# santi-pdp/segan_pytorch

Hardware: AMD Instinct MI355X
Metric: 16384-sample waveform chunks/sec (GAN step) (higher is better)
Workload: dtype f32

## Files before the change

include/segan_hip.h:

```cpp
#ifndef SEGAN_HIP_H
#define SEGAN_HIP_H

#include <stddef.h>
#include <stdint.h>

#ifdef __cplusplus
extern "C" {
#endif

#define SEGAN_ABI_VERSION 13

#define SEGAN_PAD_REFLECT 0
#define SEGAN_PAD_ZERO 1

#define SEGAN_ACT_NONE 0
#define SEGAN_ACT_TANH 1

typedef struct segan_src {
  const float* p0;
  const float* p1;
  int32_t C0;
  int32_t C1;
  const float* scale;
  const float* shift;
  const float* slope;
} segan_src;

int segan_abi_version(void);
const char* segan_last_error(void);

int segan_set_reserved_slots(int n);

size_t segan_packed_f_bytes(int M, int N, int S);
// ... 82 lines not shown
int segan_gemm(const float* A, int64_t sam, int64_t sak, const float* B, int64_t sbk, int64_t sbn,
               float* C, int64_t ldc, int M, int N, int K, int beta0, int flags, void* scratch,
               size_t scratch_bytes, void* stream);

int segan_bias_prelu_rows(const float* x, const float* bias, const float* slope, float* y,
                          int rows, int cols, void* stream);
int segan_bias_prelu_rows_bwd(const float* x, const float* bias, const float* slope,
                              const float* dy, float* dx, float* dslope, float* dbias, int rows,
                              int cols, void* stream);

int segan_mse_const(const float* x, float target, float* loss, float* grad, const float* gout,
                    float gscale, int n, void* stream);
int segan_bce_logits_const(const float* x, float target, float* loss, float* grad,
                           const float* gout, float gscale, int n, void* stream);
int segan_l1_mean(const float* x, const float* y, float* loss, float* ws, int64_t n,
                  void* stream);
int segan_l1_bwd(const float* x, const float* y, const float* gout, float gscale, float* grad,
                 int64_t n, void* stream);

size_t segan_packed_g_bytes(int M, int N, int S);
int segan_pack_weights_g(const float* w, float* wg, int M, int N, int K, int S, void* stream);
int segan_conv1d_dgrad_short(const float* da, const float* wg, float* dx, int B, int N, int M,
                             int L, int K, int S, int padL, int roll, void* stream);

int segan_pool_time_fwd(const float* x, float* y, int* idx, int rows, int L, int mode,
                        void* stream);
int segan_pool_time_bwd(const float* dy, const int* idx, float* dx, int rows, int L, int mode,
                        void* stream);

int segan_mse_mean(const float* x, const float* y, float* loss, float* ws, int64_t n,
                   void* stream);
int segan_mse_bwd(const float* x, const float* y, const float* gout, float gscale, float* grad,
                  int64_t n, void* stream);

size_t segan_snorm_ws_floats(int A, int Bd, int K, int dim);
int segan_snorm_fwd(const float* w, float* u, float* v, float* w_sn, float* sigma, float* ws, int A,
                    int Bd, int K, int dim, int power_iteration, float eps, void* stream);
int segan_snorm_bwd(const float* dw_sn, const float* w, const float* u, const float* v,
                    const float* sigma, float* dw, float* ws, int A, int Bd, int K, int dim,
                    void* stream);

int segan_stft_pitch(int n_fft);
int segan_stft_basis(float* basis, int n_fft, int win, void* stream);
int segan_stft_frames(const float* x, float* frames, int B, int T, int n_fft, int hop, int win,
                      void* stream);
int segan_powdb(const float* S, float* db, int64_t rows, int nbins, int pitch, float eps,
// ... 36 lines not shown
```

segan_pytorch_amd/_lib.py:

```python
import ctypes
import os
from ctypes import POINTER, Structure, c_char_p, c_double, c_float, c_int, c_int32, c_int64, c_size_t, c_void_p

_HERE = os.path.dirname(os.path.abspath(__file__))
LIB_PATH = os.environ.get('SEGAN_HIP_LIB') or os.path.join(_HERE, 'libsegan_hip.so')

PAD_REFLECT = 0
PAD_ZERO = 1
ACT_NONE = 0
ACT_TANH = 1
ABI_VERSION = 13


class SeganSrc(Structure):
    _fields_ = [('p0', c_void_p), ('p1', c_void_p), ('C0', c_int32), ('C1', c_int32),
                ('scale', c_void_p), ('shift', c_void_p), ('slope', c_void_p)]


_P = c_void_p
_SRC = POINTER(SeganSrc)

SIGNATURES = {
    'segan_abi_version': (c_int, []),
    'segan_set_reserved_slots': (c_int, [c_int]),
    'segan_last_error': (c_char_p, []),
    'segan_packed_f_bytes': (c_size_t, [c_int, c_int, c_int]),
    'segan_packed_t_bytes': (c_size_t, [c_int, c_int, c_int]),
    'segan_pack_weights': (c_int, [_P, _P, _P, c_int, c_int, c_int, c_int, c_int, _P]),
    'segan_packed_bf_bytes': (c_size_t, [c_int, c_int, c_int, c_int, c_int]),
    'segan_pack_weights_bf': (c_int, [_P, _P, c_int, c_int, c_int, c_int, c_int, c_int, c_int, _P]),
    'segan_corr_scratch_bytes': (c_size_t, []),
    'segan_bf16_scratch_bytes': (c_size_t, [c_int] * 9),
    'segan_debug_last_corr': (None, [POINTER(c_int)]),
    'segan_debug_last_wgrad': (None, [POINTER(c_int)]),
# ... 14 lines not shown
    'segan_bn_partial': (c_int, [_P, _P, c_int, c_int, c_int, _P]),
    'segan_bn_final': (c_int, [_P, c_int, _P, _P, c_float, c_float, _P, _P, _P, _P, _P, _P, c_int, _P]),
    'segan_act_bwd_bn_reduce': (c_int, [_P] * 12 + [c_int, c_int, c_int, _P]),
    'segan_act_bwd_bn_apply': (c_int, [_P] * 11 + [c_int, c_int, c_int, c_double, _P]),
    'segan_affine_prelu': (c_int, [_P, _P, _P, _P, _P, c_int, c_int, c_int, _P]),
    'segan_affine_tanh': (c_int, [_P, _P, _P, _P, c_int, c_int, c_int, _P]),
    'segan_scale_mask': (c_int, [_P, _P, _P, _P, c_int, c_int, c_int, _P]),
    'segan_sum_skip': (c_int, [_P, _P, _P, _P, _P, c_int, c_int, c_int, _P]),
    'segan_bce_logits_const': (c_int, [_P, c_float, _P, _P, _P, c_float, c_int, _P]),
    'segan_act_bwd': (c_int, [_P] * 16 + [c_int, c_int, c_int, _P]),
    'segan_tanh_bwd': (c_int, [_P, _P, _P, c_float, _P, _P, _P, c_int, c_int, c_int, _P]),
    'segan_gemm_scratch_bytes': (c_size_t, [c_int, c_int, c_int]),
    'segan_gemm': (c_int, [_P, c_int64, c_int64, _P, c_int64, c_int64, _P, c_int64, c_int, c_int,
                           c_int, c_int, c_int, _P, c_size_t, _P]),
    'segan_bias_prelu_rows': (c_int, [_P, _P, _P, _P, c_int, c_int, _P]),
    'segan_bias_prelu_rows_bwd': (c_int, [_P, _P, _P, _P, _P, _P, _P, c_int, c_int, _P]),
    'segan_mse_const': (c_int, [_P, c_float, _P, _P, _P, c_float, c_int, _P]),
    'segan_l1_bwd': (c_int, [_P, _P, _P, c_float, _P, c_int64, _P]),
    'segan_l1_mean': (c_int, [_P, _P, _P, _P, c_int64, _P]),
    'segan_packed_g_bytes': (c_size_t, [c_int, c_int, c_int]),
    'segan_pack_weights_g': (c_int, [_P, _P, c_int, c_int, c_int, c_int, _P]),
    'segan_conv1d_dgrad_short': (c_int, [_P, _P, _P, c_int, c_int, c_int, c_int, c_int, c_int, c_int,
                                        c_int, _P]),
    'segan_pool_time_fwd': (c_int, [_P, _P, _P, c_int, c_int, c_int, _P]),
    'segan_pool_time_bwd': (c_int, [_P, _P, _P, c_int, c_int, c_int, _P]),
    'segan_mse_mean': (c_int, [_P, _P, _P, _P, c_int64, _P]),
    'segan_mse_bwd': (c_int, [_P, _P, _P, c_float, _P, c_int64, _P]),
    'segan_snorm_ws_floats': (c_size_t, [c_int, c_int, c_int, c_int]),
    'segan_snorm_fwd': (c_int, [_P, _P, _P, _P, _P, _P, c_int, c_int, c_int, c_int, c_int, c_float, _P]),
    'segan_snorm_bwd': (c_int, [_P, _P, _P, _P, _P, _P, _P, c_int, c_int, c_int, c_int, _P]),
    'segan_pcm16_prep': (c_int, [_P, _P, _P, _P, c_int, c_int, c_double, _P]),
    'segan_stft_basis': (c_int, [_P, c_int, c_int, _P]),
    'segan_stft_frames': (c_int, [_P, _P, c_int, c_int, c_int, c_int, c_int, _P]),
    'segan_stft_pitch': (c_int, [c_int]),
    'segan_powdb': (c_int, [_P, _P, c_int64, c_int, c_int, c_float, _P]),
    'segan_powdb_bwd': (c_int, [_P, _P, _P, c_int64, c_int, c_int, c_float, _P]),
    'segan_stft_overlap_add': (c_int, [_P, _P, c_int, c_int, c_int, c_int, c_int, _P]),
    'segan_deemphasis': (c_int, [_P, _P, c_int, c_int, c_double, _P]),
    'segan_ssnr_frames': (c_int, [c_int, c_int]),
    'segan_ssnr': (c_int, [_P, _P, _P, _P, c_int, c_int, c_int, c_double, _P]),
    'segan_rmsprop_step': (c_int, [_P, _P, _P, c_float, c_float, c_float, c_int64, _P]),
    'segan_adam_step': (c_int, [_P, _P, _P, _P, c_float, c_float, c_float, c_float, c_int, c_int64,
                                _P]),
    'segan_fill': (c_int, [_P, c_float, c_int64, _P]),
    'segan_scale': (c_int, [_P, c_float, c_int64, _P]),
    'segan_comm_id_bytes': (c_int, []),
# ... 46 lines not shown
```

segan_pytorch_amd/csrc/segan_common.h:

```cpp
#pragma once
#include <hip/hip_runtime.h>
#include <stdint.h>
#include <stdio.h>
#include <stdarg.h>
#include "../../include/segan_hip.h"

#define SEGAN_OK 0
#define SEGAN_EINVAL (-1)
#define SEGAN_ELAUNCH (-2)
#define SEGAN_EUNSUPPORTED (-3)

void segan_set_error(const char* fmt, ...);
int segan_check_launch(const char* what);

#define SEGAN_REQUIRE(cond, ...)                 \
  do {                                           \
    if (!(cond)) {                               \
      segan_set_error(__VA_ARGS__);              \
      return SEGAN_EINVAL;                       \
    }                                            \
  } while (0)

typedef float f32x16 __attribute__((ext_vector_type(16)));
typedef float f32x4 __attribute__((ext_vector_type(4)));
// ... 42 lines not shown
  float sc, sh, sl;
};

__device__ __forceinline__ ChanXf segan_chan_xf(const segan_src& s, int c) {
  ChanXf x;
  x.sc = s.scale[c];
  x.sh = s.shift[c];
  x.sl = s.slope[c];
  return x;
}

__device__ __forceinline__ float segan_apply_xf(const ChanXf& x, float v) {
  v = fmaf(v, x.sc, x.sh);
  return v > 0.0f ? v : v * x.sl;
}

int segan_src_defaults(segan_src* s, hipStream_t st, const char* what);

__device__ __forceinline__ const float* segan_src_row(const segan_src& s, int b, int n, int L) {
  if (n < s.C0) return s.p0 + ((size_t)b * s.C0 + n) * (size_t)L;
  return s.p1 + ((size_t)b * s.C1 + (n - s.C0)) * (size_t)L;
}

__device__ __forceinline__ float warp_sum(float v) {
#pragma unroll
  for (int o = 32; o > 0; o >>= 1) v += __shfl_down(v, o, 64);
  return v;
}
```

segan_pytorch_amd/csrc/segan_conv.hip:

```cpp
#include "segan_conv_shared.h"

template <int MB, int NB, int WM, int U>
struct TileGeom {
  static constexpr int S = 32 / U;
  static constexpr int WN = 4 / WM;
  static constexpr int NI = MB / (32 * WM);
  static constexpr int NJ = NB / (32 * WN);
  static constexpr int NPT = MB / S;
};

struct TileWork {
  int tile, c0, c1;
  bool partial;
  int piece;
};

struct TileIter {
  int tileA;
  long unit, unit_end;
  int first_tile;
  __device__ __forceinline__ void init(const CorrArgs& a, int nch) {
    tileA = blockIdx.x;
    unit = (long)blockIdx.x * a.sk_units;
    unit_end = min(unit + (long)a.sk_units, a.sk_total);
// ... 886 lines not shown
    return;
  }
  const int row = blockIdx.x * blockDim.x + threadIdx.x;
  if (row >= rows) return;
  float* d = dx + (size_t)row * L;
  const float* hrow = halo + (size_t)row * hl;
  for (int P = 0; P < padL; ++P) {
    const int idx = segan_hi_index(P, L, padL, SEGAN_PAD_REFLECT, roll);
    if (idx >= 0) d[idx] += hrow[P];
  }
  for (int P2 = 0; P2 < padR; ++P2) {
    const int idx = segan_hi_index(L + padL + P2, L, padL, SEGAN_PAD_REFLECT, roll);
    if (idx >= 0) d[idx] += hrow[padL + P2];
  }
}

#define CS_KC 16
struct ShortArgs {
  const float* da;
  const float* wg;
  float* dx;
  int B, N, M, L, Ls, padL, padRw, roll, ncoltiles;
  int xr8, xbc;
};

template <int S>
__global__ __launch_bounds__(256, 2) void conv_dgrad_short_kernel(const ShortArgs a) {
  constexpr int MB = 128, NB = 128, KC = CS_KC, NI = 2, NJ = 2, YP = 65, U = 32 / S;
  extern __shared__ __attribute__((aligned(16))) float smem[];
  float* Wl0 = smem;
  float* Il0 = smem + 2 * KC * MB;
  const int tid = threadIdx.x;
  const int lane = tid & 63;
  const int wave = __builtin_amdgcn_readfirstlane(tid >> 6);
  const int wm = wave >> 1, wn = wave & 1;
  const int l31 = lane & 31, h = lane >> 5;
  int rowtile, coltile;
  if (a.xbc > 0) {
    const int x = blockIdx.x & 7, k = blockIdx.x >> 3;
    const int per = a.xr8 * a.xbc;
    const int cb = k / per, rem = k - cb * per;
    const int wdt = min(a.xbc, a.ncoltiles - cb * a.xbc);
    const int rr = rem / wdt;
    rowtile = x * a.xr8 + rr;
    coltile = cb * a.xbc + rem - rr * wdt;
  } else {
    const int vb = xcd_remap(blockIdx.x, gridDim.x);
    rowtile = vb / a.ncoltiles;
    coltile = vb - rowtile * a.ncoltiles;
// ... 30 lines not shown

  int aoff[NI], boff[NJ], rsh[NI];
#pragma unroll
  for (int i = 0; i < NI; ++i) {
    aoff[i] = h * MB + 32 * (wm * NI + i) + l31;
    rsh[i] = 0;
  }
#pragma unroll
  for (int j = 0; j < NJ; ++j) boff[j] = h * NB + 64 * wn + 32 * j + l31;

  f32x16 acc[NI][NJ];
#pragma unroll
  for (int i = 0; i < NI; ++i)
#pragma unroll
    for (int j = 0; j < NJ; ++j)
#pragma unroll
      for (int e = 0; e < 16; ++e) acc[i][j][e] = 0.0f;

  const int nch = a.M / KC;
  float b30_unused[NJ] = {};
  load_chunk(0, 0);
  __builtin_amdgcn_s_waitcnt(0x0f70);
  __syncthreads();
  for (int ch = 0; ch < nch; ++ch) {
    const int buf = ch & 1;
    if (ch + 1 < nch) load_chunk(ch + 1, buf ^ 1);
    corr_mma_chunk<MB, 1, KC, NI, NJ, false>(Wl0 + buf * (KC * MB), Il0 + buf * (KC * NB), NB, aoff,
                                             boff, rsh, acc, b30_unused, h, aoff, boff);
    __builtin_amdgcn_s_waitcnt(0x0f70);
    __syncthreads();
  }

  float* Yb = smem + wave * (32 * YP);
  const int bw = b0 + (64 * wn) / Ls;
  auto dxp = [&](int P, int cbase) -> float {
    const int r = P % S, qq = P / S;
    float v = 0.0f;
#pragma unroll
    for (int u = 0; u < U; ++u) {
      const int t = qq - u;
      if (t >= 0 && t < Ls) v += Yb[(r * U + u) * YP + cbase + t];
    }
    return v;
  };
#pragma unroll
  for (int i = 0; i < NI; ++i) {
#pragma unroll
    for (int j = 0; j < NJ; ++j)
#pragma unroll
      for (int e = 0; e < 16; ++e)
        Yb[((e & 3) + 8 * (e >> 2) + 4 * h) * YP + 32 * j + l31] = acc[i][j][e];
    __syncthreads();
    const int n = n0 + 2 * wm + i;
#pragma unroll
    for (int p = 0; p < S; ++p) {
      const int o = p * 64 + lane;
      const int sl = o / L, io = o - sl * L;
      const int b = bw + sl;
      float v = dxp(io + a.padL, sl * Ls);
      if (io >= 1 && io <= a.padL) v += dxp(a.padL - io, sl * Ls);
      const int jr = L - 2 - io;
      if (jr >= 0 && jr < a.padRw) v += dxp(L + a.padL + jr, sl * Ls);
      if (b < a.B && n < a.N) {
        int ii = io - a.roll;
        if (ii < 0) ii += L;
        if (ii >= L) ii -= L;
        a.dx[((size_t)b * a.N + n) * L + ii] = v;
      }
    }
    __syncthreads();
  }
}

__global__ void pack_g_kernel(const float* __restrict__ w, float* __restrict__ wg, int M, int N,
                              int K, int S) {
  const size_t total = (size_t)M * N * 32;
  const int U = 32 / S;
  for (size_t i = blockIdx.x * (size_t)blockDim.x + threadIdx.x; i < total;
       i += (size_t)gridDim.x * blockDim.x) {
    const int c = (int)(i & 31);
    const size_t mn = i >> 5;
    const int k = S * (c % U) + c / U;
    wg[i] = k < K ? w[mn * K + k] : 0.0f;
  }
}

static thread_local int g_last_corr[6];
void segan_note_corr_launch(int kind, unsigned grid, const CorrArgs& a, int ntiles) {
  g_last_corr[0] = kind;
  g_last_corr[1] = (int)grid;
  g_last_corr[2] = ntiles;
  g_last_corr[3] = a.sk_nfull;
  g_last_corr[4] = a.sk_total > 0 ? a.sk_units : 0;
// ... 463 lines not shown
  if (!stride_ok(S) || L % S != 0) return false;
  const int Ls = L / S;
  return (Ls == 4 || Ls == 8 || Ls == 16 || Ls == 32 || Ls == 64) && N % 4 == 0 &&
         M % CS_KC == 0 && K >= 1 && K <= 32 && padL >= 0 && K - 1 - padL >= 0 && padL < L &&
         K - S - padL < L;
}

extern "C" size_t segan_packed_g_bytes(int M, int N, int S) {
  if (!stride_ok(S) || M <= 0 || N <= 0) return 0;
  return (size_t)M * N * 32 * sizeof(float);
}

extern "C" int segan_pack_weights_g(const float* w, float* wg, int M, int N, int K, int S,
                                    void* stream) {
  SEGAN_REQUIRE(w && wg && M > 0 && N > 0, "pack_weights_g: bad arguments");
  SEGAN_REQUIRE(stride_ok(S) && K >= 1 && K <= 32, "pack_weights_g: stride in {1,2,4}, K <= 32");
  const size_t total = (size_t)M * N * 32;
  const int blocks = (int)((total + 255) / 256 > 8192 ? 8192 : (total + 255) / 256);
  hipLaunchKernelGGL(pack_g_kernel, dim3(blocks), dim3(256), 0, (hipStream_t)stream, w, wg, M, N, K,
                     S);
  return segan_check_launch("pack_weights_g");
}

extern "C" int segan_conv1d_dgrad_short(const float* da, const float* wg, float* dx, int B, int N,
                                        int M, int L, int K, int S, int padL, int roll,
                                        void* stream) {
  SEGAN_REQUIRE(da && wg && dx && B > 0, "conv1d_dgrad_short: bad arguments");
  SEGAN_REQUIRE(roll > -L && roll < L, "conv1d_dgrad_short: |roll| must be < L");
  if (!short_ok(N, M, L, K, S, padL)) {
    segan_set_error("conv1d_dgrad_short: geometry not covered (L/S in {4,8,16,32,64}, N %% 4 == 0, "
                    "M %% 16 == 0)");
    return SEGAN_EUNSUPPORTED;
  }
  ShortArgs a;
  a.da = da; a.wg = wg; a.dx = dx;
  a.B = B; a.N = N; a.M = M; a.L = L; a.Ls = L / S; a.padL = padL;
  a.padRw = K - S - padL > 0 ? K - S - padL : 0;
  a.roll = roll;
  a.ncoltiles = ceil_div(B, 128 / a.Ls);
  const size_t lds = 4 * 32 * 65 * sizeof(float);
  const dim3 grid((unsigned)(N / 4 * a.ncoltiles));
  static const bool blocked = [] {
    const char* e = getenv("SEGAN_SHORT_ORDER");
    return !(e && e[0] == '0');
  }();
  a.xr8 = a.xbc = 0;
  if (blocked && (N / 4) % 8 == 0) {
    a.xr8 = N / 4 / 8;
    a.xbc = a.xr8 >= 128 ? 1 : 128 / a.xr8;
  }
  hipStream_t st = (hipStream_t)stream;
  if (S == 4) hipLaunchKernelGGL(conv_dgrad_short_kernel<4>, grid, dim3(256), lds, st, a);
  else if (S == 2) hipLaunchKernelGGL(conv_dgrad_short_kernel<2>, grid, dim3(256), lds, st, a);
  else hipLaunchKernelGGL(conv_dgrad_short_kernel<1>, grid, dim3(256), lds, st, a);
  return segan_check_launch("conv_dgrad_short_kernel");
}
```

segan_pytorch_amd/csrc/segan_pointwise.hip:

```cpp
#include "segan_common.h"

#define PW_THREADS 256

static int pw_nsplit(int B, int C, int L) {
  int ns = ceil_div(2048, C);
  if (ns > B) ns = B;
  long per = (long)B * L / ns;
  while (ns > 1 && per < 2048) {
    ns = (ns + 1) / 2;
    per = (long)B * L / ns;
  }
  return ns < 1 ? 1 : ns;
}

extern "C" int segan_bn_nsplit(int B, int C, int L) {
  if (B <= 0 || C <= 0 || L <= 0) return 0;
  return pw_nsplit(B, C, L);
}

template <int NV>
__device__ __forceinline__ void block_sum(float (&v)[NV], float* sm) {
  const int lane = threadIdx.x & 63, wave = threadIdx.x >> 6;
#pragma unroll
  for (int k = 0; k < NV; ++k) v[k] = warp_sum(v[k]);
// ... 77 lines not shown
    const float r = s1 / n;
    mean = K + r;
    m2 = fmaxf(s2 - s1 * r, 0.0f);
  }
#pragma unroll
  for (int o = 32; o > 0; o >>= 1) {
    const float nb2 = __shfl_down(n, o, 64), mb2 = __shfl_down(mean, o, 64), qb2 = __shfl_down(m2, o, 64);
    chan_combine(n, mean, m2, nb2, mb2, qb2);
  }
  const int lane = threadIdx.x & 63, wave = threadIdx.x >> 6;
  if (lane == 0) {
    sm[3 * wave] = n; sm[3 * wave + 1] = mean; sm[3 * wave + 2] = m2;
  }
  __syncthreads();
  if (threadIdx.x == 0) {
    for (int w = 1; w < PW_THREADS / 64; ++w) chan_combine(n, mean, m2, sm[3 * w], sm[3 * w + 1], sm[3 * w + 2]);
    float* w = ws + ((size_t)blockIdx.y * C + cr.c) * 3;
    w[0] = n;
    w[1] = mean;
    w[2] = m2;
  }
}

__device__ __forceinline__ void bn_affine(float gamma, float beta, float mean, float rstd,
                                          float& scale, float& shift) {
  scale = gamma * rstd;
  shift = fmaf(-mean, scale, beta);
}

__global__ void bn_final_kernel(const float* __restrict__ ws, const float* gamma, const float* beta,
                                float eps, float momentum, float* running_mean, float* running_var,
                                float* mean_o, float* rstd_o, float* scale_o, float* shift_o, int C,
                                int nsplit) {
  const int c = blockIdx.x * blockDim.x + threadIdx.x;
  if (c >= C) return;
  double n = 0.0, mean = 0.0, m2 = 0.0;
  for (int s = 0; s < nsplit; ++s) {
    const float* w = ws + ((size_t)s * C + c) * 3;
    const double nb = w[0], mb = w[1], qb = w[2];
    if (nb <= 0.0) continue;
    const double tot = n + nb;
    const double d = mb - mean;
    mean += d * nb / tot;
    m2 += qb + d * d * n * nb / tot;
    n = tot;
  }
  const double var = n > 0 ? m2 / n : 0.0;
  const float rstd = (float)(1.0 / sqrt(var + (double)eps));
  const float g = gamma ? gamma[c] : 1.0f;
  const float bt = beta ? beta[c] : 0.0f;
  float sc, sh;
// ... 761 lines not shown
```

segan_pytorch_amd/distributed.py:

```python
import os
import time

import torch
import torch.distributed as dist

from . import ops


def is_dist():
    return dist.is_available() and dist.is_initialized() and dist.get_world_size() > 1


def world_size():
    return dist.get_world_size() if (dist.is_available() and dist.is_initialized()) else 1


def _collectives_on():
    if not (dist.is_available() and dist.is_initialized()):
        return False
    return dist.get_world_size() > 1 or os.environ.get('SEGAN_DP_SINGLE') == '1'


def rank():
    return dist.get_rank() if (dist.is_available() and dist.is_initialized()) else 0
# ... 436 lines not shown
    if n % ws != 0:
        raise ValueError('global batch {} is not divisible by world size {}'.format(n, ws))
    per = n // ws
    return t.narrow(dim, rk * per, per)


def sync_bn_enabled():
    return _collectives_on() and os.environ.get("SEGAN_SYNC_BN", "0") == "1"


def bn_stats_sync(x, gamma, beta, eps, momentum, running_mean, running_var):
    ws = ops.bn_partial(x)
    if _native_cur is not None:
        allp = _native_cur.allgather(ws).view(-1, ws.shape[1], 3)
    else:
        parts = [torch.empty_like(ws) for _ in range(world_size())]
        dist.all_gather(parts, ws)
        allp = torch.cat(parts, 0).contiguous()
    return ops.bn_final(allp, gamma, beta, eps, momentum, running_mean, running_var)


def act_bwd_bn_sync(a, dh, slope, bn, dslope=None, dgamma=None, dbeta=None, dbias=None):
    totals, ws = ops.act_bwd_bn_reduce(a, dh, slope, bn, dslope, dgamma, dbeta)
    if _native_cur is not None:
        _native_cur.allreduce(totals, 1.0)
    else:
        dist.all_reduce(totals, op=dist.ReduceOp.SUM)
    count = float(a.shape[0]) * float(a.shape[2]) * world_size()
    return ops.act_bwd_bn_apply(a, dh, slope, bn, totals, count, dbias, ws)
```

segan_pytorch_amd/functional.py:

```python
import os

import torch

from . import ops
from .ops import ACT_NONE, ACT_TANH, PAD_REFLECT, PAD_ZERO, Src


def grad_buf(p):
    if p.grad is None:
        p.grad = torch.zeros_like(p, memory_format=torch.contiguous_format)
    elif not p.grad.is_contiguous():
        p.grad = p.grad.contiguous()
    return p.grad


def _gb(p, needed=True):
    if p is None or not needed or not p.requires_grad:
        return None
    return grad_buf(p)


def _bn_batch_stats(bn, training):
    return training or bn.running_mean is None or bn.running_var is None

# ... 18 lines not shown
    rstd = torch.rsqrt(bn.running_var + bn.eps)
    gamma = bn.weight.detach() if bn.weight is not None else torch.ones_like(rstd)
    beta = bn.bias.detach() if bn.bias is not None else torch.zeros_like(rstd)
    scale = (gamma * rstd).contiguous()
    shift = (beta - bn.running_mean * scale).contiguous()
    return scale, shift, rstd.contiguous()


def _eval_bn_act_bwd(c, bn, scale, shift, rstd, dh, slope, dslope, y_tanh=None, dbias=None):
    if y_tanh is not None:
        g = ops.tanh_bwd(y_tanh, dh, dbias=_gb(bn.bias))
    else:
        v = ops.affine_prelu(c, scale, shift, None)
        g = ops.act_bwd(v, dh, slope=slope, dslope=dslope, dbias=_gb(bn.bias))
    if bn.weight is not None and bn.weight.requires_grad:
        xhat = ops.affine_prelu(c, rstd, (-bn.running_mean * rstd).contiguous(), None)
        grad_buf(bn.weight).add_((g * xhat).sum((0, 2)))
    dc = ops.affine_prelu(g, scale, None, None)
    if dbias is not None:
        ops.act_bwd(dc, dc, dbias=dbias)
    return dc


def _act_bwd_bn(a, dh, slope, bn, dslope, dgamma, dbeta, dbias):
    from . import distributed as sdist
    if sdist.sync_bn_enabled():
        return sdist.act_bwd_bn_sync(a, dh, slope, bn, dslope, dgamma, dbeta, dbias)
    return ops.act_bwd(a, dh, slope=slope, bn=bn, dslope=dslope, dgamma=dgamma, dbeta=dbeta,
                       dbias=dbias)


_WGRAD_OVERLAP = os.environ.get('SEGAN_WGRAD_OVERLAP', '0') == '1'
_side_streams = {}


class _SideStream(object):

    def __init__(self, *tensors):
        flat = []
        for t in tensors:
            if isinstance(t, Src):
                flat.extend((t.t0, t.t1, t.scale, t.shift, t.slope))
            else:
                flat.append(t)
        self.tensors = [t for t in flat if torch.is_tensor(t) and t.is_cuda]
        self.on = _WGRAD_OVERLAP and bool(self.tensors)

    def __enter__(self):
        if not self.on:
            return self
        dev = self.tensors[0].device
        main = torch.cuda.current_stream(dev)
# ... 323 lines not shown
                _ready(blk)
            if is_conv:
                d_in = ops.conv1d_dgrad(da, w, src.L, S, pack=blk._pack)
                if li == 0:
                    dh_last_enc = d_in if gen.no_z else d_in[:, src.C0:].contiguous()
                else:
                    dh = d_in
            elif li == 0:
                if gen.no_z:
                    _d0, dh_last_enc = ops.deconv1d_dgrad(da, w, S, 0, pack=blk._pack)
                else:
                    _d0, dh_last_enc = ops.deconv1d_dgrad(da, w, S, src.C0, need0=False,
                                                          pack=blk._pack)
            else:
                if src.C1 > 0:
                    dh, dsk = ops.deconv1d_dgrad(da, w, S, src.C0, pack=blk._pack)
                    dskip[n_enc - 1 - li] = dsk
                else:
                    _d0, dh = ops.deconv1d_dgrad(da, w, S, 0, pack=blk._pack)
                    if getattr(src, 'sum_of', False):
                        dskip[n_enc - 1 - li] = dh
        dh = dh_last_enc
        dx = None
        for l in range(n_enc - 1, -1, -1):
            blk = enc[l]
            w = W.get(blk.conv)
            K, S = blk.kwidth, blk.stride
            bnsv = bn_enc[l]
            bnm = getattr(blk, 'norm', None)
            sc, sh = xf_enc[l]
            gskip = gen.skips[l]['alpha'] if (gen.skip and l in gen.skips) else None
            dsk = dskip.get(l)
            mask, a_norm = skip_saved.get(l, (None, None))
            if dsk is not None and mask is not None:
                dsk = ops.scale_mask(dsk, None, mask)
            alpha_p = None
            if gskip is not None and gskip.skip_type == 'conv':
                if dsk is not None:
                    dsk = _skip_conv_bwd(gskip, dsk, Src(a_enc[l], scale=sc, shift=sh), W)
                alpha_v = _ones(a_enc[l].shape[1], a_enc[l]) if dsk is not None else None
                ready_extra = gskip.skip_k
            else:
                alpha_p = gskip.skip_k if gskip is not None else None
                alpha_v = alpha_p if dsk is not None else None
                ready_extra = alpha_p
            if bnsv is None:
                da = ops.act_bwd(a_enc[l], dh, dskip=dsk, slope=blk.act.weight, alpha=alpha_v,
                                 dslope=_gb(blk.act.weight),
                                 dalpha=_gb(alpha_p, dsk is not None),
                                 dbias=_gb(blk.conv.bias))
            elif dsk is None:
                da = _act_bwd_bn(a_enc[l], dh, blk.act.weight, bnsv, _gb(blk.act.weight),
                                 _gb(bnm.weight), _gb(bnm.bias), _gb(blk.conv.bias))
            else:
                if a_norm is None:
                    a_norm = ops.affine_prelu(a_enc[l], sc, sh, None)
                g = ops.act_bwd(a_norm, dh, dskip=dsk, slope=blk.act.weight, alpha=alpha_v,
                                dslope=_gb(blk.act.weight), dalpha=_gb(alpha_p, True))
                da = _act_bwd_bn(a_enc[l], g, None, bnsv, None, _gb(bnm.weight), _gb(bnm.bias),
                                 _gb(blk.conv.bias))
            padL = ops.conv_pad(K, S)[0]
            with _SideStream(da, src_enc[l]):
                if W.needs_grad(blk.conv):
                    gw = W.grad_target(blk.conv)
                    ops.wgrad(Src(da), src_enc[l], gw, K, S, padL, PAD_REFLECT)
                    W.finish(blk.conv, gw)
                _ready(blk, ready_extra)
            if l > 0:
                dh = ops.conv1d_dgrad(da, w, src_enc[l].L, S, pack=blk._pack)
            elif ctx.x_needs:
                dx = ops.conv1d_dgrad(da, w, src_enc[l].L, S, pack=blk._pack)
        _join_side(dy)
        ctx.state = None
        return (None, None, dx, None) + (None,) * (len(ctx.needs_input_grad) - 4)


class DiscriminatorFn(torch.autograd.Function):

    @staticmethod
    def forward(ctx, disc, rolls, x, x1, *params):
        x = x.contiguous()
        blocks = list(disc.enc_blocks)
        training = disc.training
        src = Src(x) if x1 is None else Src(x, x1.contiguous())
        cs, srcs, bns, xfs = [], [], [], []
        W = _Weights()
        for l, blk in enumerate(blocks):
            c = ops.conv1d_fwd(src, W.get(blk.conv), blk.conv.bias, blk.stride, roll=rolls[l],
                               pack=blk._pack)
            srcs.append(src)
            cs.append(c)
            if blk.norm is not None:
# ... 78 lines not shown
            dh = ops.linear_dgrad(dy1, W.get(fc[0])).view(cs[-1].shape)
            _ready(fc)
        else:
            h, hp, idx, y3 = head
            Lh = h.shape[2]
            dy3 = ops.bias_prelu_rows_bwd(y3, fc.bias, None, dout, None, _gb(fc.bias))
            lin_wgrad(fc, dy3, hp)
            dhp = ops.linear_dgrad(dy3, W.get(fc))
            if disc.pool_type == 'conv':
                pcm = disc.pool_conv
                dpc = dhp.view(h.shape[0], 1, Lh)
                if pcm.bias is not None and pcm.bias.requires_grad:
                    ops.act_bwd(dpc, dpc, dbias=grad_buf(pcm.bias))
                if W.needs_grad(pcm):
                    gw = W.grad_target(pcm)
                    ops.wgrad(Src(dpc), Src(h), gw, 1, 1, 0, PAD_ZERO)
                    W.finish(pcm, gw)
                dh = ops.conv1d_dgrad(dpc, W.get(pcm), Lh, 1, padL=0, pack=disc._pool_pack)
                _ready(fc, pcm)
            else:
                dh = ops.pool_time_bwd(dhp, idx, Lh, 'max' if disc.pool_type == 'gmax' else 'avg')
                _ready(fc)
        dx = None
        for l in range(len(blocks) - 1, -1, -1):
            blk = blocks[l]
            w = W.get(blk.conv)
            K, S = blk.kwidth, blk.stride
            bn = bns[l]
            if bn == 'eval':
                raise RuntimeError('Discriminator backward in eval() mode with BatchNorm is not '
                                   'supported; call .train() (the reference never does this)')
            if bn is not None:
                dc = _act_bwd_bn(cs[l], dh, blk.act.weight, bn, _gb(blk.act.weight), _gb(bn[2]),
                                 _gb(bn[3]), _gb(blk.conv.bias))
            else:
                dc = ops.act_bwd(cs[l], dh, slope=blk.act.weight, dslope=_gb(blk.act.weight),
                                 dbias=_gb(blk.conv.bias))
            padL = ops.conv_pad(K, S)[0]
            with _SideStream(dc, srcs[l]):
                if W.needs_grad(blk.conv):
                    gw = W.grad_target(blk.conv)
                    ops.wgrad(Src(dc), srcs[l], gw, K, S, padL, PAD_REFLECT, roll=ctx.rolls[l])
                    W.finish(blk.conv, gw)
                _ready(blk)
            if l > 0:
                dh = ops.conv1d_dgrad(dc, w, srcs[l].L, S, roll=ctx.rolls[l], pack=blk._pack)
            elif ctx.x_needs:
                dx = ops.conv1d_dgrad(dc, w, srcs[l].L, S, roll=ctx.rolls[l], pack=blk._pack)
        _join_side(dout)
        ctx.state = None
        dx1 = None
        if dx is not None and ctx.split is not None:
            c0, need0, need1 = ctx.split
            dx1 = dx[:, c0:].contiguous() if need1 else None
            dx = dx[:, :c0].contiguous() if need0 else None
        return (None, None, dx, dx1) + (None,) * (len(ctx.needs_input_grad) - 4)


class ConvBlockFn(torch.autograd.Function):

    @staticmethod
    def forward(ctx, blk, x, *params):
        x = x.contiguous()
        src = Src(x)
        W = _Weights()
        c = ops.conv1d_fwd(src, W.get(blk.conv), blk.conv.bias, blk.stride, pack=blk._pack)
        bn_saved = None
        scale = shift = None
        if blk.norm is not None:
# ... 206 lines not shown
```

segan_pytorch_amd/ops.py:

```python
import ctypes

import torch

from . import _lib
from . import layout
from ._lib import ACT_NONE, ACT_TANH, PAD_REFLECT, PAD_ZERO, SeganSrc, check


import os as _os

PREC_FP32, PREC_BF16, PREC_BF16X3 = 0, 1, 3
_PREC_NAMES = {'fp32': PREC_FP32, 'bf16': PREC_BF16, 'bf16x3': PREC_BF16X3}
_precision = _PREC_NAMES[_os.environ.get('SEGAN_PRECISION', 'fp32')]
_EUNSUPPORTED = -3


_deterministic = _os.environ.get('SEGAN_DETERMINISTIC', '0') == '1'


def set_deterministic(on):
    global _deterministic
    _deterministic = bool(on)


# ... 319 lines not shown
    if short_rows_ok(N, M, L, S):
        return conv1d_dgrad_short(da, w, L, S, roll=roll, padL=padL, pack=pack)
    check(lib.segan_conv1d_dgrad(_ptr(da), _ptr(pack.t(w, S, 0)), None, _ptr(dx), _ptr(halo), B, N,
                                 M, L, K, S, padL, roll, _fp32(), *_scratch(), _stream()),
          'conv1d_dgrad')
    return dx


def conv1d_dgrad_short(da, w, L, S, roll=0, padL=None, pack=None):
    _chk(da, 'da', 3)
    _chk(w, 'weight', 3)
    M, N, K = w.shape
    B = da.shape[0]
    if padL is None:
        padL = conv_pad(K, S)[0]
    dx = torch.empty((B, N, L), device=da.device, dtype=torch.float32)
    pack = pack or WeightPack()
    check(_lib.load().segan_conv1d_dgrad_short(_ptr(da), _ptr(pack.g(w, S)), _ptr(dx), B, N,
                                               M, L, K, S, padL, roll, _stream()),
          'conv1d_dgrad_short')
    return dx


_SHORT_LS = (4, 8, 16, 32, 64)


def short_rows_ok(N, M, L, S):
    return S in (2, 4) and L % S == 0 and (L // S) in _SHORT_LS and N % 4 == 0 and M % 16 == 0


def wgrad(lo, hi, dw, K, S, padL, pad_mode, roll=0):
    _chk(dw, 'dw', 3)
    M, N = lo.C, hi.C
    if tuple(dw.shape) != (M, N, K):
        raise ValueError('wgrad: dw {} != ({}, {}, {})'.format(tuple(dw.shape), M, N, K))
    if lo.B != hi.B or lo.L * S != hi.L:
        raise ValueError('wgrad: lo [{}x{}] / hi [{}x{}] inconsistent for stride {}'.format(
            lo.B, lo.L, hi.B, hi.L, S))
    cl, ch = lo.c_struct(), hi.c_struct()
    lib = _lib.load()
    if _precision != PREC_FP32:
        nbytes = lib.segan_wgrad_scratch_bytes(lo.B, M, N, lo.L, S, _precision, 0)
        scratch = _stream_scratch(nbytes, dw.device)
        rc = lib.segan_wgrad(ctypes.byref(cl), ctypes.byref(ch), _ptr(dw), lo.B, M, N, lo.L, K, S,
                             padL, pad_mode, roll, _precision, 0,
                             ctypes.c_void_p(scratch.data_ptr()) if scratch is not None else None,
# ... 564 lines not shown
```

Measured before the change: 3577.

## Fuse PReLU/BatchNorm backward epilogue into short-row dgrad kernel

Adds an epilogue to the short-row transposed-conv dgrad kernel. It applies the previous layer's PReLU (with optional skip tap) or BatchNorm-PReLU backward right after the output is computed. Per-channel partial sums for dslope, dalpha, dbias, dgamma and dbeta are written to a workspace, and a small final kernel reduces them. The encoder and discriminator backward loops now route eligible layers through this path, so the separate activation-backward pass that re-reads the gradient tensor is skipped. In exchange the kernel gains extra register pressure and an extra launch, and it only applies to fp32 short-row shapes.

```diff
diff --git a/include/segan_hip.h b/include/segan_hip.h
--- a/include/segan_hip.h
+++ b/include/segan_hip.h
@@ -8,7 +8,7 @@
 extern "C" {
 #endif
 
-#define SEGAN_ABI_VERSION 13
+#define SEGAN_ABI_VERSION 14
 
 #define SEGAN_PAD_REFLECT 0
 #define SEGAN_PAD_ZERO 1
@@ -137,6 +137,14 @@
 int segan_pack_weights_g(const float* w, float* wg, int M, int N, int K, int S, void* stream);
 int segan_conv1d_dgrad_short(const float* da, const float* wg, float* dx, int B, int N, int M,
                              int L, int K, int S, int padL, int roll, void* stream);
+size_t segan_short_act_ws_floats(int B, int N, int L, int S);
+int segan_conv1d_dgrad_short_act(const float* da, const float* wg, float* dx, int B, int N, int M,
+                                 int L, int K, int S, int padL, int roll, const float* a,
+                                 const float* dskip, const float* slope, const float* alpha,
+                                 const float* bn_mean, const float* bn_rstd,
+                                 const float* bn_gamma, const float* bn_beta, float* dslope,
+                                 float* dalpha, float* dgamma, float* dbeta, float* dbias,
+                                 float* totals, float* ws, void* stream);
 
 int segan_pool_time_fwd(const float* x, float* y, int* idx, int rows, int L, int mode,
                         void* stream);
diff --git a/segan_pytorch_amd/_lib.py b/segan_pytorch_amd/_lib.py
--- a/segan_pytorch_amd/_lib.py
+++ b/segan_pytorch_amd/_lib.py
@@ -9,7 +9,7 @@
 PAD_ZERO = 1
 ACT_NONE = 0
 ACT_TANH = 1
-ABI_VERSION = 13
+ABI_VERSION = 14
 
 
 class SeganSrc(Structure):
@@ -70,6 +70,8 @@
     'segan_pack_weights_g': (c_int, [_P, _P, c_int, c_int, c_int, c_int, _P]),
     'segan_conv1d_dgrad_short': (c_int, [_P, _P, _P, c_int, c_int, c_int, c_int, c_int, c_int, c_int,
                                         c_int, _P]),
+    'segan_short_act_ws_floats': (c_size_t, [c_int, c_int, c_int, c_int]),
+    'segan_conv1d_dgrad_short_act': (c_int, [_P, _P, _P] + [c_int] * 8 + [_P] * 15 + [_P]),
     'segan_pool_time_fwd': (c_int, [_P, _P, _P, c_int, c_int, c_int, _P]),
     'segan_pool_time_bwd': (c_int, [_P, _P, _P, c_int, c_int, c_int, _P]),
     'segan_mse_mean': (c_int, [_P, _P, _P, _P, c_int64, _P]),
diff --git a/segan_pytorch_amd/csrc/segan_common.h b/segan_pytorch_amd/csrc/segan_common.h
--- a/segan_pytorch_amd/csrc/segan_common.h
+++ b/segan_pytorch_amd/csrc/segan_common.h
@@ -88,6 +88,12 @@
   return s.p1 + ((size_t)b * s.C1 + (n - s.C0)) * (size_t)L;
 }
 
+__device__ __forceinline__ void bn_affine(float gamma, float beta, float mean, float rstd,
+                                          float& scale, float& shift) {
+  scale = gamma * rstd;
+  shift = fmaf(-mean, scale, beta);
+}
+
 __device__ __forceinline__ float warp_sum(float v) {
 #pragma unroll
   for (int o = 32; o > 0; o >>= 1) v += __shfl_down(v, o, 64);
diff --git a/segan_pytorch_amd/csrc/segan_conv.hip b/segan_pytorch_amd/csrc/segan_conv.hip
--- a/segan_pytorch_amd/csrc/segan_conv.hip
+++ b/segan_pytorch_amd/csrc/segan_conv.hip
@@ -932,9 +932,11 @@
   float* dx;
   int B, N, M, L, Ls, padL, padRw, roll, ncoltiles;
   int xr8, xbc;
+  const float *ea, *eskip, *eslope, *ealpha, *emean, *erstd, *egamma, *ebeta;
+  float* epart;
 };
 
-template <int S>
+template <int S, int EPI = 0>
 __global__ __launch_bounds__(256, 2) void conv_dgrad_short_kernel(const ShortArgs a) {
   constexpr int MB = 128, NB = 128, KC = CS_KC, NI = 2, NJ = 2, YP = 65, U = 32 / S;
   extern __shared__ __attribute__((aligned(16))) float smem[];
@@ -1011,6 +1013,40 @@
   load_chunk(0, 0);
   __builtin_amdgcn_s_waitcnt(0x0f70);
   __syncthreads();
+  const int bw = b0 + (64 * wn) / Ls;
+  auto out_off = [&](int i, int p) -> long {
+    const int n = n0 + 2 * wm + i;
+    const int o = p * 64 + lane;
+    const int sl = o / L, io = o - sl * L;
+    const int b = bw + sl;
+    if (b >= a.B || n >= a.N) return -1;
+    int ii = io - a.roll;
+    if (ii < 0) ii += L;
+    if (ii >= L) ii -= L;
+    return ((long)b * a.N + n) * L + ii;
+  };
+  float ev[NI][S], ek[NI][S], csl[NI], cal[NI], cmu[NI], crs[NI], csc[NI], csh[NI];
+  auto epi_load = [&]() {
+#pragma unroll
+    for (int i = 0; i < NI; ++i) {
+      const int n = n0 + 2 * wm + i;
+      csl[i] = a.eslope ? a.eslope[n] : 1.0f;
+      cal[i] = a.ealpha ? a.ealpha[n] : 0.0f;
+      cmu[i] = 0.f; crs[i] = 1.f; csc[i] = 1.f; csh[i] = 0.f;
+      if (EPI == 2) {
+        cmu[i] = a.emean[n];
+        crs[i] = a.erstd[n];
+        bn_affine(a.egamma ? a.egamma[n] : 1.0f, a.ebeta ? a.ebeta[n] : 0.0f, cmu[i], crs[i], csc[i],
+                  csh[i]);
+      }
+#pragma unroll
+      for (int p = 0; p < S; ++p) {
+        const long off = out_off(i, p);
+        ev[i][p] = off >= 0 ? a.ea[off] : 0.0f;
+        ek[i][p] = (EPI == 1 && a.eskip && off >= 0) ? a.eskip[off] : 0.0f;
+      }
+    }
+  };
   for (int ch = 0; ch < nch; ++ch) {
     const int buf = ch & 1;
     if (ch + 1 < nch) load_chunk(ch + 1, buf ^ 1);
@@ -1020,8 +1056,8 @@
     __syncthreads();
   }
 
+  if (EPI != 0) epi_load();
   float* Yb = smem + wave * (32 * YP);
-  const int bw = b0 + (64 * wn) / Ls;
   auto dxp = [&](int P, int cbase) -> float {
     const int r = P % S, qq = P / S;
     float v = 0.0f;
@@ -1040,7 +1076,9 @@
       for (int e = 0; e < 16; ++e)
         Yb[((e & 3) + 8 * (e >> 2) + 4 * h) * YP + 32 * j + l31] = acc[i][j][e];
     __syncthreads();
+    if (EPI != 0 && i == 0) __builtin_amdgcn_s_waitcnt(0x0f70);
     const int n = n0 + 2 * wm + i;
+    float r[3] = {0.f, 0.f, 0.f};
 #pragma unroll
     for (int p = 0; p < S; ++p) {
       const int o = p * 64 + lane;
@@ -1054,10 +1092,72 @@
         int ii = io - a.roll;
         if (ii < 0) ii += L;
         if (ii >= L) ii -= L;
+        const float av = ev[i][p];
+        if (EPI == 1) {
+          float g = v * (av > 0.f ? 1.0f : csl[i]);
+          r[0] += v * (av > 0.f ? 0.0f : av);
+          if (a.eskip) {
+            g = fmaf(cal[i], ek[i][p], g);
+            r[1] = fmaf(ek[i][p], av, r[1]);
+          }
+          r[2] += g;
+          v = g;
+        } else if (EPI == 2) {
+          const float xh = (av - cmu[i]) * crs[i];
+          const float vv = fmaf(av, csc[i], csh[i]);
+          const float g = v * (vv > 0.f ? 1.0f : csl[i]);
+          r[0] += v * (vv > 0.f ? 0.0f : vv);
+          r[1] += g;
+          r[2] = fmaf(g, xh, r[2]);
+        }
         a.dx[((size_t)b * a.N + n) * L + ii] = v;
       }
     }
+    if (EPI != 0) {
+#pragma unroll
+      for (int k = 0; k < 3; ++k) r[k] = warp_sum(r[k]);
+      if (lane == 0) {
+        float* w = a.epart + ((size_t)(coltile * 2 + wn) * 3) * a.N + n;
+        w[0] = r[0];
+        w[a.N] = r[1];
+        w[2 * a.N] = r[2];
+      }
+    }
     __syncthreads();
+  }
+}
+
+template <int EPI>
+__global__ __launch_bounds__(256) void short_act_final_kernel(const float* __restrict__ part,
+                                                              int nslots, int N, float* dslope,
+                                                              float* d1, float* d2, float* totals) {
+  __shared__ float sm[3][16][17];
+  const int cl = threadIdx.x & 15, t = threadIdx.x >> 4;
+  const int c = blockIdx.x * 16 + cl;
+  float s[3] = {0.f, 0.f, 0.f};
+  if (c < N)
+    for (int k = t; k < nslots; k += 16)
+#pragma unroll
+      for (int q = 0; q < 3; ++q) s[q] += part[((size_t)k * 3 + q) * N + c];
+#pragma unroll
+  for (int q = 0; q < 3; ++q) sm[q][t][cl] = s[q];
+  __syncthreads();
+  for (int w = 8; w > 0; w >>= 1) {
+    if (t < w)
+#pragma unroll
+      for (int q = 0; q < 3; ++q) sm[q][t][cl] += sm[q][t + w][cl];
+    __syncthreads();
+  }
+  if (t != 0 || c >= N) return;
+#pragma unroll
+  for (int q = 0; q < 3; ++q) s[q] = sm[q][0][cl];
+  const float o0 = dslope ? dslope[c] : 0.f, o1 = d1 ? d1[c] : 0.f, o2 = d2 ? d2[c] : 0.f;
+  if (dslope) dslope[c] = o0 + s[0];
+  if (d1) d1[c] = o1 + s[1];
+  if (d2) d2[c] = o2 + s[2];
+  if (EPI == 2) {
+    totals[2 * c] = s[1];
+    totals[2 * c + 1] = s[2];
   }
 }
 
@@ -1567,9 +1667,14 @@
   return segan_check_launch("pack_weights_g");
 }
 
-extern "C" int segan_conv1d_dgrad_short(const float* da, const float* wg, float* dx, int B, int N,
-                                        int M, int L, int K, int S, int padL, int roll,
-                                        void* stream) {
+struct ShortEpi {
+  const float *a, *dskip, *slope, *alpha, *mean, *rstd, *gamma, *beta;
+  float *dslope, *dalpha, *dgamma, *dbeta, *dbias, *totals, *part;
+};
+
+static int conv1d_dgrad_short(const float* da, const float* wg, float* dx, int B, int N, int M,
+                              int L, int K, int S, int padL, int roll, int epi,
+                              const ShortEpi* epi_args, void* stream) {
   SEGAN_REQUIRE(da && wg && dx && B > 0, "conv1d_dgrad_short: bad arguments");
   SEGAN_REQUIRE(roll > -L && roll < L, "conv1d_dgrad_short: |roll| must be < L");
   if (!short_ok(N, M, L, K, S, padL)) {
@@ -1594,9 +1699,64 @@
     a.xr8 = N / 4 / 8;
     a.xbc = a.xr8 >= 128 ? 1 : 128 / a.xr8;
   }
+  a.ea = a.eskip = a.eslope = a.ealpha = a.emean = a.erstd = a.egamma = a.ebeta = nullptr;
+  a.epart = nullptr;
   hipStream_t st = (hipStream_t)stream;
-  if (S == 4) hipLaunchKernelGGL(conv_dgrad_short_kernel<4>, grid, dim3(256), lds, st, a);
-  else if (S == 2) hipLaunchKernelGGL(conv_dgrad_short_kernel<2>, grid, dim3(256), lds, st, a);
-  else hipLaunchKernelGGL(conv_dgrad_short_kernel<1>, grid, dim3(256), lds, st, a);
-  return segan_check_launch("conv_dgrad_short_kernel");
-}
+  if (epi == 0) {
+    if (S == 4) hipLaunchKernelGGL((conv_dgrad_short_kernel<4, 0>), grid, dim3(256), lds, st, a);
+    else if (S == 2) hipLaunchKernelGGL((conv_dgrad_short_kernel<2, 0>), grid, dim3(256), lds, st, a);
+    else hipLaunchKernelGGL((conv_dgrad_short_kernel<1, 0>), grid, dim3(256), lds, st, a);
+    return segan_check_launch("conv_dgrad_short_kernel");
+  }
+  const ShortEpi& e = *epi_args;
+  a.ea = e.a; a.eskip = e.dskip; a.eslope = e.slope; a.ealpha = e.alpha;
+  a.emean = e.mean; a.erstd = e.rstd; a.egamma = e.gamma; a.ebeta = e.beta;
+  a.epart = e.part;
+  if (epi == 1) {
+    if (S == 4) hipLaunchKernelGGL((conv_dgrad_short_kernel<4, 1>), grid, dim3(256), lds, st, a);
+    else if (S == 2) hipLaunchKernelGGL((conv_dgrad_short_kernel<2, 1>), grid, dim3(256), lds, st, a);
+    else hipLaunchKernelGGL((conv_dgrad_short_kernel<1, 1>), grid, dim3(256), lds, st, a);
+    hipLaunchKernelGGL(short_act_final_kernel<1>, dim3(ceil_div(N, 16)), dim3(256), 0, st, e.part,
+                       2 * a.ncoltiles, N, e.dslope, e.dalpha, e.dbias, (float*)nullptr);
+  } else {
+    if (S == 4) hipLaunchKernelGGL((conv_dgrad_short_kernel<4, 2>), grid, dim3(256), lds, st, a);
+    else if (S == 2) hipLaunchKernelGGL((conv_dgrad_short_kernel<2, 2>), grid, dim3(256), lds, st, a);
+    else hipLaunchKernelGGL((conv_dgrad_short_kernel<1, 2>), grid, dim3(256), lds, st, a);
+    hipLaunchKernelGGL(short_act_final_kernel<2>, dim3(ceil_div(N, 16)), dim3(256), 0, st, e.part,
+                       2 * a.ncoltiles, N, e.dslope, e.dbeta, e.dgamma, e.totals);
+  }
+  return segan_check_launch("conv_dgrad_short_kernel (fused epilogue)");
+}
+
+extern "C" int segan_conv1d_dgrad_short(const float* da, const float* wg, float* dx, int B, int N,
+                                        int M, int L, int K, int S, int padL, int roll,
+                                        void* stream) {
+  return conv1d_dgrad_short(da, wg, dx, B, N, M, L, K, S, padL, roll, 0, nullptr, stream);
+}
+
+extern "C" size_t segan_short_act_ws_floats(int B, int N, int L, int S) {
+  if (B <= 0 || N <= 0 || S <= 0 || L % S != 0 || L / S <= 0 || 128 % (L / S) != 0) return 0;
+  return (size_t)2 * ceil_div(B, 128 / (L / S)) * 3 * N;
+}
+
+extern "C" int segan_conv1d_dgrad_short_act(const float* da, const float* wg, float* dx, int B,
+                                            int N, int M, int L, int K, int S, int padL, int roll,
+                                            const float* a, const float* dskip, const float* slope,
+                                            const float* alpha, const float* bn_mean,
+                                            const float* bn_rstd, const float* bn_gamma,
+                                            const float* bn_beta, float* dslope, float* dalpha,
+                                            float* dgamma, float* dbeta, float* dbias,
+                                            float* totals, float* ws, void* stream) {
+  SEGAN_REQUIRE(a && ws, "conv1d_dgrad_short_act: NULL pointer");
+  SEGAN_REQUIRE((bn_mean == nullptr) == (bn_rstd == nullptr), "conv1d_dgrad_short_act: mean/rstd must pair");
+  SEGAN_REQUIRE(!(dskip && !alpha), "conv1d_dgrad_short_act: dskip needs alpha");
+  SEGAN_REQUIRE(!(bn_mean && (dskip || dalpha || dbias)),
+                "conv1d_dgrad_short_act: BatchNorm layers take no skip tap and no bias here");
+  SEGAN_REQUIRE(!bn_mean || totals, "conv1d_dgrad_short_act: BatchNorm needs totals");
+  ShortEpi e;
+  e.a = a; e.dskip = dskip; e.slope = slope; e.alpha = alpha;
+  e.mean = bn_mean; e.rstd = bn_rstd; e.gamma = bn_gamma; e.beta = bn_beta;
+  e.dslope = dslope; e.dalpha = dalpha; e.dgamma = dgamma; e.dbeta = dbeta; e.dbias = dbias;
+  e.totals = totals; e.part = ws;
+  return conv1d_dgrad_short(da, wg, dx, B, N, M, L, K, S, padL, roll, bn_mean ? 2 : 1, &e, stream);
+}
diff --git a/segan_pytorch_amd/csrc/segan_pointwise.hip b/segan_pytorch_amd/csrc/segan_pointwise.hip
--- a/segan_pytorch_amd/csrc/segan_pointwise.hip
+++ b/segan_pytorch_amd/csrc/segan_pointwise.hip
@@ -123,11 +123,6 @@
   }
 }
 
-__device__ __forceinline__ void bn_affine(float gamma, float beta, float mean, float rstd,
-                                          float& scale, float& shift) {
-  scale = gamma * rstd;
-  shift = fmaf(-mean, scale, beta);
-}
 
 __global__ void bn_final_kernel(const float* __restrict__ ws, const float* gamma, const float* beta,
                                 float eps, float momentum, float* running_mean, float* running_var,
diff --git a/segan_pytorch_amd/distributed.py b/segan_pytorch_amd/distributed.py
--- a/segan_pytorch_amd/distributed.py
+++ b/segan_pytorch_amd/distributed.py
@@ -482,6 +482,10 @@
 
 def act_bwd_bn_sync(a, dh, slope, bn, dslope=None, dgamma=None, dbeta=None, dbias=None):
     totals, ws = ops.act_bwd_bn_reduce(a, dh, slope, bn, dslope, dgamma, dbeta)
+    return act_bwd_bn_apply_sync(a, dh, slope, bn, totals, dbias, ws)
+
+
+def act_bwd_bn_apply_sync(a, dh, slope, bn, totals, dbias=None, ws=None):
     if _native_cur is not None:
         _native_cur.allreduce(totals, 1.0)
     else:
diff --git a/segan_pytorch_amd/functional.py b/segan_pytorch_amd/functional.py
--- a/segan_pytorch_amd/functional.py
+++ b/segan_pytorch_amd/functional.py
@@ -64,12 +64,31 @@
     return dc
 
 
+def _enc_fusable(gen, l, bn_enc, skip_saved):
+    if bn_enc[l] is not None:
+        return False, None
+    gskip = gen.skips[l]['alpha'] if (gen.skip and l in gen.skips) else None
+    if gskip is None:
+        return True, None
+    if gskip.skip_type == 'conv' or skip_saved.get(l, (None, None))[0] is not None:
+        return False, None
+    return True, gskip.skip_k
+
+
 def _act_bwd_bn(a, dh, slope, bn, dslope, dgamma, dbeta, dbias):
     from . import distributed as sdist
     if sdist.sync_bn_enabled():
         return sdist.act_bwd_bn_sync(a, dh, slope, bn, dslope, dgamma, dbeta, dbias)
     return ops.act_bwd(a, dh, slope=slope, bn=bn, dslope=dslope, dgamma=dgamma, dbeta=dbeta,
                        dbias=dbias)
+
+
+def _act_bwd_bn_apply(a, dh, slope, bn, totals, dbias):
+    from . import distributed as sdist
+    if sdist.sync_bn_enabled():
+        return sdist.act_bwd_bn_apply_sync(a, dh, slope, bn, totals, dbias)
+    return ops.act_bwd_bn_apply(a, dh, slope, bn, totals, float(a.shape[0]) * float(a.shape[2]),
+                                dbias)
 
 
 _WGRAD_OVERLAP = os.environ.get('SEGAN_WGRAD_OVERLAP', '0') == '1'
@@ -439,6 +458,7 @@
                         dskip[n_enc - 1 - li] = dh
         dh = dh_last_enc
         dx = None
+        fused_da = None
         for l in range(n_enc - 1, -1, -1):
             blk = enc[l]
             w = W.get(blk.conv)
@@ -461,7 +481,9 @@
                 alpha_p = gskip.skip_k if gskip is not None else None
                 alpha_v = alpha_p if dsk is not None else None
                 ready_extra = alpha_p
-            if bnsv is None:
+            if fused_da is not None:
+                da, fused_da = fused_da, None
+            elif bnsv is None:
                 da = ops.act_bwd(a_enc[l], dh, dskip=dsk, slope=blk.act.weight, alpha=alpha_v,
                                  dslope=_gb(blk.act.weight),
                                  dalpha=_gb(alpha_p, dsk is not None),
@@ -484,7 +506,16 @@
                     W.finish(blk.conv, gw)
                 _ready(blk, ready_extra)
             if l > 0:
-                dh = ops.conv1d_dgrad(da, w, src_enc[l].L, S, pack=blk._pack)
+                fusable, pv = _enc_fusable(gen, l - 1, bn_enc, skip_saved)
+                if fusable and ops.fused_dgrad_ok(da, w, src_enc[l].L, S):
+                    bp = enc[l - 1]
+                    dsk_p = dskip.get(l - 1)
+                    fused_da, _t = ops.conv1d_dgrad_act(
+                        da, w, src_enc[l].L, S, a_enc[l - 1], slope=bp.act.weight, dskip=dsk_p,
+                        alpha=pv if dsk_p is not None else None, dslope=_gb(bp.act.weight),
+                        dalpha=_gb(pv, dsk_p is not None), dbias=_gb(bp.conv.bias), pack=blk._pack)
+                else:
+                    dh = ops.conv1d_dgrad(da, w, src_enc[l].L, S, pack=blk._pack)
             elif ctx.x_needs:
                 dx = ops.conv1d_dgrad(da, w, src_enc[l].L, S, pack=blk._pack)
         _join_side(dy)
@@ -609,6 +640,7 @@
                 dh = ops.pool_time_bwd(dhp, idx, Lh, 'max' if disc.pool_type == 'gmax' else 'avg')
                 _ready(fc)
         dx = None
+        totals = None
         for l in range(len(blocks) - 1, -1, -1):
             blk = blocks[l]
             w = W.get(blk.conv)
@@ -617,7 +649,10 @@
             if bn == 'eval':
                 raise RuntimeError('Discriminator backward in eval() mode with BatchNorm is not '
                                    'supported; call .train() (the reference never does this)')
-            if bn is not None:
+            if totals is not None:
+                dc = _act_bwd_bn_apply(cs[l], dh, blk.act.weight, bn, totals, _gb(blk.conv.bias))
+                totals = None
+            elif bn is not None:
                 dc = _act_bwd_bn(cs[l], dh, blk.act.weight, bn, _gb(blk.act.weight), _gb(bn[2]),
                                  _gb(bn[3]), _gb(blk.conv.bias))
             else:
@@ -631,7 +666,15 @@
                     W.finish(blk.conv, gw)
                 _ready(blk)
             if l > 0:
-                dh = ops.conv1d_dgrad(dc, w, srcs[l].L, S, roll=ctx.rolls[l], pack=blk._pack)
+                bnp = bns[l - 1]
+                if isinstance(bnp, tuple) and ops.fused_dgrad_ok(dc, w, srcs[l].L, S):
+                    bp = blocks[l - 1]
+                    dh, totals = ops.conv1d_dgrad_act(
+                        dc, w, srcs[l].L, S, cs[l - 1], slope=bp.act.weight, bn=bnp,
+                        dslope=_gb(bp.act.weight), dgamma=_gb(bnp[2]), dbeta=_gb(bnp[3]),
+                        roll=ctx.rolls[l], pack=blk._pack)
+                else:
+                    dh = ops.conv1d_dgrad(dc, w, srcs[l].L, S, roll=ctx.rolls[l], pack=blk._pack)
             elif ctx.x_needs:
                 dx = ops.conv1d_dgrad(dc, w, srcs[l].L, S, roll=ctx.rolls[l], pack=blk._pack)
         _join_side(dout)
diff --git a/segan_pytorch_amd/ops.py b/segan_pytorch_amd/ops.py
--- a/segan_pytorch_amd/ops.py
+++ b/segan_pytorch_amd/ops.py
@@ -365,6 +365,58 @@
     return dx
 
 
+_fused_epilogue = _os.environ.get('SEGAN_FUSED_EPILOGUE', '1') != '0'
+
+
+def set_fused_epilogue(on):
+    global _fused_epilogue
+    _fused_epilogue = bool(on)
+
+
+def get_fused_epilogue():
+    return _fused_epilogue
+
+
+def fused_dgrad_ok(da, w, L, S):
+    M, N, K = w.shape
+    return (_fused_epilogue and not _precision and isinstance(da, torch.Tensor) and da.is_cuda
+            and N > 2 and short_rows_ok(N, M, L, S))
+
+
+def conv1d_dgrad_act(da, w, L, S, a, slope=None, dskip=None, alpha=None, bn=None, dslope=None,
+                     dalpha=None, dgamma=None, dbeta=None, dbias=None, roll=0, padL=None,
+                     pack=None):
+    _chk(da, 'da', 3)
+    _chk(w, 'weight', 3)
+    _chk(a, 'a', 3)
+    M, N, K = w.shape
+    B = da.shape[0]
+    if da.shape[1] != M or da.shape[2] * S != L or tuple(a.shape) != (B, N, L):
+        raise ValueError('conv1d_dgrad_act: da {} / a {} inconsistent with weight {} / L {}'.format(
+            tuple(da.shape), tuple(a.shape), tuple(w.shape), L))
+    if dskip is not None:
+        _chk(dskip, 'dskip', 3)
+        if dskip.shape != a.shape:
+            raise ValueError('conv1d_dgrad_act: dskip {} vs a {}'.format(tuple(dskip.shape),
+                                                                         tuple(a.shape)))
+    if padL is None:
+        padL = conv_pad(K, S)[0]
+    pack = pack or WeightPack()
+    lib = _lib.load()
+    out = torch.empty((B, N, L), device=da.device, dtype=torch.float32)
+    ws = _stream_scratch(4 * lib.segan_short_act_ws_floats(B, N, L, S), da.device)
+    mean = rstd = gamma = beta = totals = None
+    if bn is not None:
+        mean, rstd, gamma, beta = bn
+        totals = torch.empty((N, 2), device=da.device, dtype=torch.float32)
+    check(lib.segan_conv1d_dgrad_short_act(
+        _ptr(da), _ptr(pack.g(w, S)), _ptr(out), B, N, M, L, K, S, padL, roll, _ptr(a),
+        _ptr(dskip), _ptr(slope), _ptr(alpha), _ptr(mean), _ptr(rstd), _ptr(gamma), _ptr(beta),
+        _ptr(dslope), _ptr(dalpha), _ptr(dgamma), _ptr(dbeta), _ptr(dbias), _ptr(totals), _ptr(ws),
+        _stream()), 'conv1d_dgrad_short_act')
+    return out, totals
+
+
 _SHORT_LS = (4, 8, 16, 32, 64)
 
 
```

Result: no change. 3572, median of 2 (-0.1%).
